# dog-qiuqiu/Yolo-FastestV2

Hardware: AMD Instinct MI355X
Metric: images/sec at 352x352 bs=256 per GPU (forward+decode+NMS) (higher is better)
Workload: dtype f32 tensors; contractions fp16x3 (two-term fp16 split operands on v_mfma_f32_16x16x32_f16, fp32 accumulate); depthwise/BN/ReLU/decode/NMS fp32 VALU; 1 GPU

## Files before the change

yolo_fastestv2_amd/csrc/yfv2_post.hip:

```cpp
#include "yfv2_internal.h"

__device__ __forceinline__ float sigmoid_f32(float x) { return __fdiv_rn(1.0f, __fadd_rn(1.0f, expf(-x))); }

template <bool SKIP = false, int MAXPER = 24>
__device__ __forceinline__ void yfv2_compact_row(const DecodeArgs& a, int b, int sc, int cc, int part, f32x4& r0, f32x4& r1,
                                                 const float (&objl)[3] = {0.f, 0.f, 0.f}, float skip_ct = 0.f) {
  const int fh = a.fh[sc], fw = a.fw[sc], hw = fh * fw;
  const int nc = a.classes;
  const int per = (nc + 3) >> 2;
  const int c_lo = part * per, c_hi = min(nc, c_lo + per);
  const float* cls = a.cls[sc] + (size_t)b * nc * hw;
  float best[3] = {0.f, 0.f, 0.f};
  int bj[3] = {0, 0, 0};
  bool need = true;
  if constexpr (SKIP) need = sigmoid_f32(objl[0]) > skip_ct || sigmoid_f32(objl[1]) > skip_ct || sigmoid_f32(objl[2]) > skip_ct;
  if (need) {
    float lv[MAXPER];
#pragma unroll
    for (int i = 0; i < MAXPER; ++i) {
      const int c = c_lo + i;
      lv[i] = cls[(unsigned)((c < c_hi ? c : (c_lo < nc ? c_lo : 0)) * hw + cc)];
    }
    float m = -INFINITY;
#pragma unroll
    for (int i = 0; i < MAXPER; ++i)
      if (c_lo + i < c_hi) m = fmaxf(m, lv[i]);
    m = fmaxf(m, __shfl_xor(m, 1));
    m = fmaxf(m, __shfl_xor(m, 2));
    float sum = 0.f;
#pragma unroll
    for (int i = 0; i < MAXPER; ++i) {
      const float e = expf(__fsub_rn(lv[i], m));
      lv[i] = e;
      if (c_lo + i < c_hi) sum = __fadd_rn(sum, e);
      if ((i & 3) == 3) __builtin_amdgcn_sched_barrier(0);
    }
    sum = __fadd_rn(sum, __shfl_xor(sum, 1));
    sum = __fadd_rn(sum, __shfl_xor(sum, 2));
    float obj3[3];
#pragma unroll
    for (int an = 0; an < 3; ++an) {
      obj3[an] = sigmoid_f32(a.obj[sc][((size_t)b * 3 + an) * hw + cc]);
      best[an] = -INFINITY;
      bj[an] = 0x7fffffff;
    }
    const float ev1 = __fdiv_rn(1.0f, sum);
    int first = 0x7fffffff, cnt = 0;
#pragma unroll
    for (int i = 0; i < MAXPER; ++i) {
      const bool near_max = c_lo + i < c_hi && lv[i] >= 0.99999904632568359375f;
      first = near_max ? min(first, c_lo + i) : first;
      cnt += near_max ? 1 : 0;
    }
    cnt += __shfl_xor(cnt, 1);
    cnt += __shfl_xor(cnt, 2);
    first = min(first, __shfl_xor(first, 1));
    first = min(first, __shfl_xor(first, 2));
    bool exact = cnt != 1;
#pragma unroll
    for (int an = 0; an < 3; ++an) {
      best[an] = __fmul_rn(ev1, obj3[an]);
      bj[an] = first;
      exact |= !(best[an] > 7.888609052210118e-31f);
    }
    if (exact) {
#pragma unroll
      for (int an = 0; an < 3; ++an) { best[an] = -INFINITY; bj[an] = 0x7fffffff; }
#pragma unroll
      for (int i = 0; i < MAXPER; ++i) {
        if (c_lo + i < c_hi) {
          const float ev = __fdiv_rn(lv[i], sum);
#pragma unroll
          for (int an = 0; an < 3; ++an) {
            const float pj = __fmul_rn(ev, obj3[an]);
            if (pj > best[an]) { best[an] = pj; bj[an] = c_lo + i; }
          }
        }
        if ((i & 3) == 3) __builtin_amdgcn_sched_barrier(0);
      }
#pragma unroll
      for (int an = 0; an < 3; ++an)
#pragma unroll
        for (int msk = 1; msk < 4; msk <<= 1) {
          const float ob_ = __shfl_xor(best[an], msk);
          const int oi = __shfl_xor(bj[an], msk);
          if (ob_ > best[an] || (ob_ == best[an] && oi < bj[an])) { best[an] = ob_; bj[an] = oi; }
        }
    }
  }
  const int an = part < 3 ? part : 0;
  const int y = cc / fw, x = cc - y * fw;
  const float* reg = a.reg[sc] + ((size_t)b * 12 + an * 4) * hw + cc;
  const float t0 = reg[0], t1 = reg[(size_t)hw], t2 = reg[(size_t)2 * hw], t3 = reg[(size_t)3 * hw];
  const float ob = a.obj[sc][((size_t)b * 3 + an) * hw + cc];
  const float st = a.stride[sc];
  const float qw = __fmul_rn(sigmoid_f32(t2), 2.0f), qh = __fmul_rn(sigmoid_f32(t3), 2.0f);
  r0 = (f32x4){__fmul_rn(__fadd_rn(__fsub_rn(__fmul_rn(sigmoid_f32(t0), 2.0f), 0.5f), (float)x), st),
               __fmul_rn(__fadd_rn(__fsub_rn(__fmul_rn(sigmoid_f32(t1), 2.0f), 0.5f), (float)y), st),
               (float)((double)__fmul_rn(qw, qw) * a.anchors[(sc * 3 + an) * 2 + 0]),
               (float)((double)__fmul_rn(qh, qh) * a.anchors[(sc * 3 + an) * 2 + 1])};
  r1 = (f32x4){sigmoid_f32(ob), part == 0 ? best[0] : (part == 1 ? best[1] : best[2]), (float)(part == 0 ? bj[0] : (part == 1 ? bj[1] : bj[2])), 0.f};
}

constexpr int DEC_CELLS = 64;
constexpr int DEC_THREADS = 256;

template <bool COMPACT, int MAXPER = 24>
__global__ __launch_bounds__(DEC_THREADS) void decode_kernel(DecodeArgs a, int blocks0, int blocks1) {
  constexpr int CELLS = MAXPER > 24 ? 32 : DEC_CELLS, THREADS = 4 * CELLS;
  extern __shared__ float stage[];
  const int per_img = blocks0 + blocks1;
  const int b = blockIdx.x / per_img;
  int blk = blockIdx.x - b * per_img;
  const int sc = blk >= blocks0 ? 1 : 0;
  if (sc) blk -= blocks0;
  const int fh = a.fh[sc], fw = a.fw[sc], hw = fh * fw;
  const int cell0 = blk * CELLS;
  const int ncell = min(CELLS, hw - cell0);
  const int nc = a.classes, rowlen = 5 + nc;
  const int tid = threadIdx.x;
  const int lc = tid >> 2, part = tid & 3;
  const int cell = cell0 + lc;
  const bool ok = lc < ncell;
  const int cc = ok ? cell : cell0;

  const int per = (nc + 3) >> 2;
  const int c_lo = part * per, c_hi = min(nc, c_lo + per);
  const float* cls = a.cls[sc] + (size_t)b * nc * hw;
  float lv[MAXPER];
#pragma unroll
  for (int i = 0; i < MAXPER; ++i) {
    const int c = c_lo + i;
    lv[i] = cls[(unsigned)((c < c_hi ? c : (c_lo < nc ? c_lo : 0)) * hw + cc)];
  }
  float m = -INFINITY;
#pragma unroll
  for (int i = 0; i < MAXPER; ++i)
    if (c_lo + i < c_hi) m = fmaxf(m, lv[i]);
  m = fmaxf(m, __shfl_xor(m, 1));
  m = fmaxf(m, __shfl_xor(m, 2));
  float sum = 0.f;
  float ev[MAXPER];
#pragma unroll
  for (int i = 0; i < MAXPER; ++i) {
    ev[i] = 0.f;
    if (c_lo + i < c_hi) {
      ev[i] = expf(__fsub_rn(lv[i], m));
      sum = __fadd_rn(sum, ev[i]);
    }
  }
  sum = __fadd_rn(sum, __shfl_xor(sum, 1));
  sum = __fadd_rn(sum, __shfl_xor(sum, 2));
#pragma unroll
  for (int i = 0; i < MAXPER; ++i) ev[i] = __fdiv_rn(ev[i], sum);

  auto box_of = [&](int an, float (&o)[5]) {
    const int y = cell / fw, x = cell - y * fw;
    const float* reg = a.reg[sc] + ((size_t)b * 12 + an * 4) * hw + cell;
    const float t0 = reg[0], t1 = reg[(size_t)hw], t2 = reg[(size_t)2 * hw], t3 = reg[(size_t)3 * hw];
    const float ob = a.obj[sc][((size_t)b * 3 + an) * hw + cell];
    const float st = a.stride[sc];
    o[0] = __fmul_rn(__fadd_rn(__fsub_rn(__fmul_rn(sigmoid_f32(t0), 2.0f), 0.5f), (float)x), st);
    o[1] = __fmul_rn(__fadd_rn(__fsub_rn(__fmul_rn(sigmoid_f32(t1), 2.0f), 0.5f), (float)y), st);
    const float qw = __fmul_rn(sigmoid_f32(t2), 2.0f), qh = __fmul_rn(sigmoid_f32(t3), 2.0f);
    o[2] = (float)((double)__fmul_rn(qw, qw) * a.anchors[(sc * 3 + an) * 2 + 0]);
    o[3] = (float)((double)__fmul_rn(qh, qh) * a.anchors[(sc * 3 + an) * 2 + 1]);
    o[4] = sigmoid_f32(ob);
  };
  const size_t row0 = (size_t)b * a.rows + (sc ? 3 * a.fh[0] * a.fw[0] : 0) + (size_t)cell0 * 3;

  if constexpr (COMPACT) {
    f32x4 r0, r1;
    yfv2_compact_row<false, MAXPER>(a, b, sc, cc, part, r0, r1);
    if (ok && part < 3) {
      float* d = a.cand + (row0 + (size_t)lc * 3 + part) * 8;
      *reinterpret_cast<f32x4*>(d) = r0;
      *reinterpret_cast<f32x4*>(d + 4) = r1;
    }
  } else {
    float* srow = stage + (size_t)lc * 3 * rowlen;
    if (ok) {
#pragma unroll
      for (int i = 0; i < MAXPER; ++i) {
        const int c = c_lo + i;
        if (c < c_hi) {
          srow[5 + c] = ev[i];
          srow[rowlen + 5 + c] = ev[i];
          srow[2 * rowlen + 5 + c] = ev[i];
        }
      }
      if (part < 3) {
        float o[5];
        box_of(part, o);
        float* d = srow + part * rowlen;
#pragma unroll
        for (int k = 0; k < 5; ++k) d[k] = o[k];
      }
    }
    __syncthreads();
    float* dst = a.boxes + row0 * rowlen;
    const int n = ncell * 3 * rowlen;
    for (int i = tid; i < n; i += THREADS) dst[i] = stage[i];
  }
}

void yfv2_launch_decode(const DecodeArgs& a, hipStream_t s) {
  const int cells = a.classes <= 96 ? DEC_CELLS : 32;
  const int b0 = (a.fh[0] * a.fw[0] + cells - 1) / cells;
  const int b1 = (a.fh[1] * a.fw[1] + cells - 1) / cells;
  const size_t lds = (size_t)cells * 3 * (5 + a.classes) * sizeof(float);
  static std::atomic<unsigned long long> lds_ok0{0}, lds_ok1{0}, lds_ok2{0}, lds_ok3{0};
  if (a.classes <= 96) {
    yfv2_allow_full_lds(reinterpret_cast<const void*>(&decode_kernel<false>), lds_ok0);
    yfv2_allow_full_lds(reinterpret_cast<const void*>(&decode_kernel<true>), lds_ok1);
    if (a.cand)
      YFV2_LAUNCH(decode_kernel<true>, dim3(a.B * (b0 + b1)), dim3(DEC_THREADS), 0, s, a, b0, b1);
    else
      YFV2_LAUNCH(decode_kernel<false>, dim3(a.B * (b0 + b1)), dim3(DEC_THREADS), lds, s, a, b0, b1);
  } else {
    yfv2_allow_full_lds(reinterpret_cast<const void*>(&decode_kernel<false, 64>), lds_ok2);
    yfv2_allow_full_lds(reinterpret_cast<const void*>(&decode_kernel<true, 64>), lds_ok3);
    if (a.cand)
      YFV2_LAUNCH((decode_kernel<true, 64>), dim3(a.B * (b0 + b1)), dim3(4 * cells), 0, s, a, b0, b1);
    else
      YFV2_LAUNCH((decode_kernel<false, 64>), dim3(a.B * (b0 + b1)), dim3(4 * cells), lds, s, a, b0, b1);
  }
}
bool yfv2_post_fusable(int classes, int rows) { return classes <= 96 && rows <= 2048; }
int yfv2_nms_max_rows() { return 4096; }

constexpr int NMS_THREADS = 1024;
constexpr int NMS_NQ = NMS_THREADS / 64;
constexpr int NMS_CAP = 2048;
constexpr int NMS_MAX_DET = 300;

#define NMS_STAMP(i) do { if (a.trace && blockIdx.x == 0 && threadIdx.x == 0) a.trace[i] = (long long)__builtin_readcyclecounter(); } while (0)
template <int SRC, int KPT = 2>
__global__ __launch_bounds__(NMS_THREADS) void nms_kernel(NmsArgs a, DecodeArgs dec) {
  constexpr bool COMPACT = SRC >= 1;
  constexpr int CAP = KPT * NMS_THREADS;
  static_assert(KPT == 2 || (KPT == 4 && SRC != 2), "two keys per thread, or four without the in-LDS decode");
  extern __shared__ __attribute__((aligned(16))) float crow[];
  __shared__ unsigned long long key[CAP];
  __shared__ __attribute__((aligned(16))) float geo[(KPT == 2 ? 7 : 5) * CAP];
  unsigned long long* const key2 = reinterpret_cast<unsigned long long*>(geo);
  float* const bx1 = geo + (KPT == 2 ? 2 * CAP : 0);
  float* const by1 = bx1 + CAP; float* const bx2 = by1 + CAP; float* const by2 = bx2 + CAP; float* const area = by2 + CAP;
  __shared__ unsigned char supp[CAP];
  __shared__ unsigned char cls_of_row[CAP];
  __shared__ int keep[NMS_MAX_DET];
  __shared__ float kx1[NMS_MAX_DET], kx2[NMS_MAX_DET];
  __shared__ unsigned long long pmask[NMS_NQ][64];
  __shared__ int n_cand, n_keep, n_obj;

  const int tid = threadIdx.x, b = blockIdx.x;
  const int rowlen = COMPACT ? 8 : 5 + a.nc;
  const float* img = SRC == 2 ? crow : a.boxes + (size_t)b * a.rows * rowlen;
  const float ct = a.conf_thres;
  NMS_STAMP(0);
  if constexpr (SRC == 2) {
    constexpr int CPP = NMS_THREADS / 4;
    const int hw0 = dec.fh[0] * dec.fw[0], hw1 = dec.fh[1] * dec.fw[1];
    const int np0 = (hw0 + CPP - 1) / CPP, np = np0 + (hw1 + CPP - 1) / CPP;
    const int part = tid & 3;
    auto obj_of = [&](int ps, float (&o)[3]) {
      const int sc = ps < np0 ? 0 : 1, hw = sc ? hw1 : hw0;
      const int cell = (ps - (sc ? np0 : 0)) * CPP + (tid >> 2);
      const int cc = cell < hw ? cell : hw - 1;
#pragma unroll
      for (int an = 0; an < 3; ++an) o[an] = ps < np ? dec.obj[sc][((size_t)b * 3 + an) * hw + cc] : 0.f;
    };
    float ocur[3], onxt[3];
    obj_of(0, ocur);
    for (int ps = 0; ps < np; ++ps) {
      obj_of(ps + 1, onxt);
      const int sc = ps < np0 ? 0 : 1, hw = sc ? hw1 : hw0;
      const int row_base = sc ? 3 * hw0 : 0;
      const int cell = (ps - (sc ? np0 : 0)) * CPP + (tid >> 2);
      const bool ok = cell < hw;
      f32x4 r0, r1;
      yfv2_compact_row<true>(dec, b, sc, ok ? cell : hw - 1, part, r0, r1, ocur, ct);
      if (ok && part < 3) {
        float* d = crow + (size_t)(row_base + cell * 3 + part) * 8;
        *reinterpret_cast<f32x4*>(d) = r0;
        *reinterpret_cast<f32x4*>(d + 4) = r1;
      }
#pragma unroll
      for (int an = 0; an < 3; ++an) ocur[an] = onxt[an];
    }
    __syncthreads();
  }
  NMS_STAMP(1);
  unsigned short* cand_row = reinterpret_cast<unsigned short*>(bx1);
  if (tid == 0) { n_cand = 0; n_keep = 0; n_obj = 0; }
  __syncthreads();

  if constexpr (COMPACT) {
    for (int n0 = 0; n0 < a.rows; n0 += NMS_THREADS) {
      const int n = n0 + tid;
      f32x4 t = {0.f, 0.f, 0.f, 0.f};
      if (n < a.rows) t = *reinterpret_cast<const f32x4*>(img + (size_t)n * 8 + 4);
      const bool pass = n < a.rows && t[0] > ct && t[1] > ct;
      const unsigned long long m = __ballot(pass);
      int base = 0;
      if ((tid & 63) == 0 && m) base = atomicAdd(&n_cand, (int)__popcll(m));
      base = __shfl(base, 0);
      if (pass) {
        const int slot = base + (int)__popcll(m & ((1ull << (tid & 63)) - 1ull));
        key[slot] = ((unsigned long long)__float_as_uint(t[1]) << 32) | (unsigned long long)(0xFFFFFFFFu - (unsigned)n);
        cls_of_row[n] = (unsigned char)(int)t[2];
      }
    }
  } else {
    for (int n0 = 0; n0 < a.rows; n0 += NMS_THREADS) {
      const int n = n0 + tid;
      const bool pass = n < a.rows && img[(size_t)n * rowlen + 4] > ct;
      const unsigned long long m = __ballot(pass);
      int base = 0;
      if ((tid & 63) == 0 && m) base = atomicAdd(&n_obj, (int)__popcll(m));
      base = __shfl(base, 0);
      if (pass) cand_row[base + (int)__popcll(m & ((1ull << (tid & 63)) - 1ull))] = (unsigned short)n;
    }
    __syncthreads();
    {
      const int l16 = tid & 15, grp = tid >> 4, ngrp = NMS_THREADS >> 4;
      const int nobj = n_obj;
      for (int q = grp; q < nobj; q += ngrp) {
        const int n = cand_row[q];
        const float* r = img + (size_t)n * rowlen;
        const float obj = r[4];
        float best = -INFINITY;
        int bj = 0x7fffffff;
        for (int j = l16; j < a.nc; j += 16) {
          const float pj = __fmul_rn(r[5 + j], obj);
          if (pj > best) { best = pj; bj = j; }
        }
#pragma unroll
        for (int m = 1; m < 16; m <<= 1) {
          const float ob = __shfl_xor(best, m, 16);
          const int oj = __shfl_xor(bj, m, 16);
          if (ob > best || (ob == best && oj < bj)) { best = ob; bj = oj; }
        }
        if (l16 == 0 && best > ct) {
          bool hit = true;
          if (a.classes) {
            hit = false;
            for (int k = 0; k < a.n_classes; ++k) hit |= (a.classes[k] == bj);
          }
          if (hit) {
            const int slot = atomicAdd(&n_cand, 1);
            key[slot] = ((unsigned long long)__float_as_uint(best) << 32) | (unsigned long long)(0xFFFFFFFFu - (unsigned)n);
            cls_of_row[n] = (unsigned char)bj;
          }
        }
      }
    }
  }
  __syncthreads();
  NMS_STAMP(2);
  const int n = n_cand;
  if (n == 0) {
    if (tid == 0) a.count[b] = 0;
    return;
  }

  int np2 = 1;
  while (np2 < n) np2 <<= 1;
  for (int i = n + tid; i < np2; i += NMS_THREADS) key[i] = 0ull;
  __syncthreads();
  if constexpr (KPT == 2) {
    static_assert(NMS_CAP == 2 * NMS_THREADS, "two keys per thread");
    const int i0 = tid, i1 = tid + NMS_THREADS;
    unsigned long long k0 = i0 < np2 ? key[i0] : 0ull, k1 = i1 < np2 ? key[i1] : 0ull;
    auto cx = [](unsigned long long x, unsigned long long y, bool take_max) { return take_max == (x > y) ? x : y; };
    int pb = 0;
    for (int k = 2; k <= np2; k <<= 1) {
      for (int j = k >> 1; j > 0; j >>= 1) {
        const bool d0 = (i0 & k) == 0, d1 = (i1 & k) == 0;
        if (j >= NMS_THREADS) {
          const unsigned long long hi = k0 > k1 ? k0 : k1, lo = k0 > k1 ? k1 : k0;
          k0 = d0 ? hi : lo; k1 = d0 ? lo : hi;
        } else if (j >= 64) {
          unsigned long long* buf = pb ? key2 : key;
          buf[i0] = k0; buf[i1] = k1;
          __syncthreads();
          const unsigned long long y0 = buf[i0 ^ j], y1 = buf[i1 ^ j];
          const bool low = (i0 & j) == 0;
          k0 = cx(k0, y0, low == d0); k1 = cx(k1, y1, low == d1);
          pb ^= 1;
        } else {
          const unsigned long long y0 = __shfl_xor(k0, j), y1 = __shfl_xor(k1, j);
          const bool low = (i0 & j) == 0;
          k0 = cx(k0, y0, low == d0); k1 = cx(k1, y1, low == d1);
        }
      }
    }
    __syncthreads();
    if (i0 < np2) key[i0] = k0;
    if (i1 < np2) key[i1] = k1;
    __syncthreads();
  } else {
    unsigned long long k[KPT];
#pragma unroll
    for (int r = 0; r < KPT; ++r) { const int i = tid + r * NMS_THREADS; k[r] = i < np2 ? key[i] : 0ull; }
    auto cx = [](unsigned long long x, unsigned long long y, bool take_max) { return take_max == (x > y) ? x : y; };
    int pb = 0;
    for (int kk = 2; kk <= np2; kk <<= 1) {
      for (int j = kk >> 1; j > 0; j >>= 1) {
        if (j >= NMS_THREADS) {
          const int jr = j / NMS_THREADS;
#pragma unroll
          for (int r = 0; r < KPT; ++r) {
            if ((r & jr) == 0) {
              const int r2 = r | jr;
              const bool desc = ((tid + r * NMS_THREADS) & kk) == 0;
              const unsigned long long hi = k[r] > k[r2] ? k[r] : k[r2], lo = k[r] > k[r2] ? k[r2] : k[r];
              k[r] = desc ? hi : lo; k[r2] = desc ? lo : hi;
            }
          }
        } else if (j >= 64) {
          unsigned long long* buf = pb ? key2 : key;
#pragma unroll
          for (int r = 0; r < KPT; ++r) buf[tid + r * NMS_THREADS] = k[r];
          __syncthreads();
          const bool low = (tid & j) == 0;
#pragma unroll
          for (int r = 0; r < KPT; ++r) {
            const int i = tid + r * NMS_THREADS;
            k[r] = cx(k[r], buf[i ^ j], low == ((i & kk) == 0));
          }
          pb ^= 1;
        } else {
          const bool low = (tid & j) == 0;
#pragma unroll
          for (int r = 0; r < KPT; ++r) {
            const int i = tid + r * NMS_THREADS;
            k[r] = cx(k[r], __shfl_xor(k[r], j), low == ((i & kk) == 0));
          }
        }
      }
    }
    __syncthreads();
#pragma unroll
    for (int r = 0; r < KPT; ++r) { const int i = tid + r * NMS_THREADS; if (i < np2) key[i] = k[r]; }
    __syncthreads();
  }

  NMS_STAMP(3);
  for (int i = tid; i < n; i += NMS_THREADS) {
    const unsigned row = 0xFFFFFFFFu - (unsigned)(key[i] & 0xFFFFFFFFull);
    const float* r = img + (size_t)row * rowlen;
    const float cx = r[0], cy = r[1], hw_ = __fdiv_rn(r[2], 2.0f), hh = __fdiv_rn(r[3], 2.0f);
    const float c = __fmul_rn((float)cls_of_row[row], 4096.0f);
    const float x1 = __fadd_rn(__fsub_rn(cx, hw_), c), y1 = __fadd_rn(__fsub_rn(cy, hh), c);
    const float x2 = __fadd_rn(__fadd_rn(cx, hw_), c), y2 = __fadd_rn(__fadd_rn(cy, hh), c);
    bx1[i] = x1; by1[i] = y1; bx2[i] = x2; by2[i] = y2;
    area[i] = __fmul_rn(__fsub_rn(x2, x1), __fsub_rn(y2, y1));
    supp[i] = 0;
  }
  __syncthreads();

  NMS_STAMP(4);
  const bool thr_nonneg = a.iou_thres >= 0.0;
  auto overlaps = [&](int i, int j) -> bool {
    const float xx1 = fmaxf(bx1[i], bx1[j]), xx2 = fminf(bx2[i], bx2[j]);
    if (thr_nonneg && !(xx2 > xx1)) return false;
    const float yy1 = fmaxf(by1[i], by1[j]), yy2 = fminf(by2[i], by2[j]);
    const float w = fmaxf(0.0f, __fsub_rn(xx2, xx1)), h = fmaxf(0.0f, __fsub_rn(yy2, yy1));
    const float inter = __fmul_rn(w, h);
    const float ovr = __fdiv_rn(inter, __fsub_rn(__fadd_rn(area[i], area[j]), inter));
    return (double)ovr > a.iou_thres;
  };
  const int j = tid & 63, q = tid >> 6;
  long long t_tests = 0, t_walk = 0, t_bar = 0; int n_chunks = 0;
  const bool tr = a.trace && blockIdx.x == 0 && tid == 0;
  for (int c0 = 0; c0 < n; c0 += 64) {
    const int nk = n_keep;
    if (nk >= NMS_MAX_DET) break;
    const long long ts0 = tr ? (long long)__builtin_readcyclecounter() : 0;
    const int m = min(64, n - c0);
    unsigned long long bits = 0ull;
    {
      constexpr int KMAX = (NMS_MAX_DET + NMS_NQ - 1) / NMS_NQ;
      constexpr int PER = 64 / NMS_NQ;
      auto lane_f = [](float v, int l) { return __builtin_bit_cast(float, __builtin_amdgcn_readlane(__builtin_bit_cast(int, v), l)); };
      const int cj = c0 + j;
      const bool live = j < m;
      const float jx1 = live ? bx1[cj] : INFINITY, jx2 = live ? bx2[cj] : -INFINITY;
      const int kl = q + NMS_NQ * j;
      const bool kv = j < KMAX && kl < nk;
      const float rk1 = kv ? kx1[kl] : INFINITY, rk2 = kv ? kx2[kl] : -INFINITY;
      unsigned cand = 0u;
#pragma unroll
      for (int t = 0; t < KMAX; ++t) {
        const float a1 = lane_f(rk1, t), a2 = lane_f(rk2, t);
        if (q + NMS_NQ * t < nk && (!thr_nonneg || fminf(a2, jx2) > fmaxf(a1, jx1))) cand |= 1u << t;
      }
      unsigned icand = 0u;
#pragma unroll
      for (int c = 0; c < PER; ++c) {
        const int i = PER * q + c;
        const float a1 = lane_f(jx1, i), a2 = lane_f(jx2, i);
        if (i < j && (!thr_nonneg || fminf(a2, jx2) > fmaxf(a1, jx1))) icand |= 1u << c;
      }
      if (live) {
        while (cand) {
          const int t = __builtin_ctz(cand);
          cand &= cand - 1u;
          if (overlaps(keep[q + NMS_NQ * t], cj)) { supp[cj] = 1; break; }
        }
        while (icand) {
          const int c = __builtin_ctz(icand);
          icand &= icand - 1u;
          if (overlaps(c0 + PER * q + c, cj)) bits |= 1ull << (PER * q + c);
        }
      }
    }
    pmask[q][j] = bits;
    const long long ts1 = tr ? (long long)__builtin_readcyclecounter() : 0;
    __syncthreads();
    const long long ts2 = tr ? (long long)__builtin_readcyclecounter() : 0;
    if (tid < 64) {
      unsigned long long S = 0ull;
#pragma unroll
      for (int qq = 0; qq < NMS_NQ; ++qq) S |= pmask[qq][tid];
      const bool alive = tid < m && !supp[c0 + tid];
      const unsigned long long alive_mask = __ballot(alive);
      unsigned long long kmask = alive_mask;
      for (int it = 0; it < 64; ++it) {
        const unsigned long long k2 = __ballot(alive && !(S & kmask));
        if (k2 == kmask) break;
        kmask = k2;
      }
      if ((kmask >> tid) & 1ull) {
        const int pos = nk + __popcll(kmask & ((1ull << tid) - 1ull));
        if (pos < NMS_MAX_DET) { keep[pos] = c0 + tid; kx1[pos] = bx1[c0 + tid]; kx2[pos] = bx2[c0 + tid]; }
      }
      if (tid == 0) n_keep = min(NMS_MAX_DET, nk + __popcll(kmask));
    }
    const long long ts3 = tr ? (long long)__builtin_readcyclecounter() : 0;
    __syncthreads();
    if (tr) { const long long ts4 = (long long)__builtin_readcyclecounter(); t_tests += ts1 - ts0; t_walk += ts3 - ts2; t_bar += (ts2 - ts1) + (ts4 - ts3); ++n_chunks; }
  }
  if (tr) { a.trace[9] = n_chunks; a.trace[10] = t_tests; a.trace[11] = t_walk; a.trace[12] = t_bar; }
  __syncthreads();
  NMS_STAMP(5);
  const int kept = n_keep;

  for (int k = tid; k < kept; k += NMS_THREADS) {
    const int i = keep[k];
    const unsigned long long kk = key[i];
    const unsigned row = 0xFFFFFFFFu - (unsigned)(kk & 0xFFFFFFFFull);
    const float* r = img + (size_t)row * rowlen;
    const float cx = r[0], cy = r[1], hw_ = __fdiv_rn(r[2], 2.0f), hh = __fdiv_rn(r[3], 2.0f);
    float* d = a.dets + ((size_t)b * NMS_MAX_DET + k) * 6;
    d[0] = __fsub_rn(cx, hw_); d[1] = __fsub_rn(cy, hh);
    d[2] = __fadd_rn(cx, hw_); d[3] = __fadd_rn(cy, hh);
    d[4] = __uint_as_float((unsigned)(kk >> 32));
    d[5] = (float)cls_of_row[row];
    a.idx[(size_t)b * NMS_MAX_DET + k] = (int)row;
  }
  if (tid == 0) a.count[b] = kept;
  NMS_STAMP(6);
  if (a.trace && blockIdx.x == 0 && tid == 0) { a.trace[7] = n; a.trace[8] = kept; }
}

void yfv2_launch_nms(const NmsArgs& a, hipStream_t s) {
  const DecodeArgs none{};
  if (a.rows <= NMS_CAP) {
    if (a.compact)
      YFV2_LAUNCH(nms_kernel<1>, dim3(a.B), dim3(NMS_THREADS), 0, s, a, none);
    else
      YFV2_LAUNCH(nms_kernel<0>, dim3(a.B), dim3(NMS_THREADS), 0, s, a, none);
  } else {
    if (a.compact)
      YFV2_LAUNCH((nms_kernel<1, 4>), dim3(a.B), dim3(NMS_THREADS), 0, s, a, none);
    else
      YFV2_LAUNCH((nms_kernel<0, 4>), dim3(a.B), dim3(NMS_THREADS), 0, s, a, none);
  }
}

void yfv2_launch_decode_nms(const DecodeArgs& d, const NmsArgs& a, hipStream_t s) {
  static std::atomic<unsigned long long> done{0};
  int dev = 0;
  if (hipGetDevice(&dev) != hipSuccess || dev < 0 || dev > 63) dev = 0;
  if (!(done.load() & (1ull << dev))) {
    (void)hipFuncSetAttribute(reinterpret_cast<const void*>(&nms_kernel<2>), hipFuncAttributeMaxDynamicSharedMemorySize, NMS_CAP * 8 * (int)sizeof(float));
    done.fetch_or(1ull << dev);
  }
  YFV2_LAUNCH(nms_kernel<2>, dim3(a.B), dim3(NMS_THREADS), (size_t)a.rows * 8 * sizeof(float), s, a, d);
}

__global__ __launch_bounds__(64) void stats_kernel(StatsArgs a) {
  __shared__ float tx1[STATS_MAX_TARGETS], ty1[STATS_MAX_TARGETS], tx2[STATS_MAX_TARGETS], ty2[STATS_MAX_TARGETS], tlab[STATS_MAX_TARGETS];
  __shared__ int tdone[STATS_MAX_TARGETS];
  const int b = blockIdx.x, lane = threadIdx.x;
  int nt = 0;
  for (int t0 = 0; t0 < a.T; t0 += 64) {
    const int t = t0 + lane;
    const bool mine = t < a.T && a.targets[(size_t)t * 6] == (float)b;
    const unsigned long long m = __ballot(mine);
    if (mine) {
      const int pos = nt + __popcll(m & ((1ull << lane) - 1ull));
      if (pos < STATS_MAX_TARGETS) {
        tlab[pos] = a.targets[(size_t)t * 6 + 1];
        tx1[pos] = a.targets[(size_t)t * 6 + 2]; ty1[pos] = a.targets[(size_t)t * 6 + 3];
        tx2[pos] = a.targets[(size_t)t * 6 + 4]; ty2[pos] = a.targets[(size_t)t * 6 + 5];
        tdone[pos] = 0;
      }
    }
    nt += __popcll(m);
  }
  if (nt > STATS_MAX_TARGETS) { if (lane == 0) *a.overflow = 1; nt = STATS_MAX_TARGETS; }
  __syncthreads();
  const int n = a.count[b];
  int* tp = a.tp + (size_t)b * NMS_MAX_DET;
  for (int i = lane; i < NMS_MAX_DET; i += 64) tp[i] = 0;
  if (nt == 0) return;
  const float thr = a.iou_thres;
  int matched = 0;
  for (int i = 0; i < n && matched < nt; ++i) {
    const float* d = a.dets + ((size_t)b * NMS_MAX_DET + i) * 6;
    const float bx1 = d[0], by1 = d[1], bx2 = d[2], by2 = d[3], lab = d[5];
    const float barea = __fmul_rn(__fadd_rn(__fsub_rn(bx2, bx1), 1.f), __fadd_rn(__fsub_rn(by2, by1), 1.f));
    bool has = false;
    float best = -1.f;
    int bidx = 0x7fffffff;
    for (int t = lane; t < nt; t += 64) {
      has |= tlab[t] == lab;
      const float ix1 = fmaxf(bx1, tx1[t]), iy1 = fmaxf(by1, ty1[t]), ix2 = fminf(bx2, tx2[t]), iy2 = fminf(by2, ty2[t]);
      const float iw = fmaxf(__fadd_rn(__fsub_rn(ix2, ix1), 1.f), 0.f), ih = fmaxf(__fadd_rn(__fsub_rn(iy2, iy1), 1.f), 0.f);
      const float inter = __fmul_rn(iw, ih);
      const float tarea = __fmul_rn(__fadd_rn(__fsub_rn(tx2[t], tx1[t]), 1.f), __fadd_rn(__fsub_rn(ty2[t], ty1[t]), 1.f));
      const float iou = __fdiv_rn(inter, __fadd_rn(__fsub_rn(__fadd_rn(barea, tarea), inter), 1e-16f));
      if (iou > best) { best = iou; bidx = t; }
    }
    if (__ballot(has) == 0ull) continue;
#pragma unroll
    for (int off = 32; off > 0; off >>= 1) {
      const float ob = __shfl_xor(best, off);
      const int oi = __shfl_xor(bidx, off);
      if (ob > best || (ob == best && oi < bidx)) { best = ob; bidx = oi; }
    }
    if (best >= thr && tdone[bidx] == 0) {
      if (lane == 0) { tp[i] = 1; tdone[bidx] = 1; }
      ++matched;
    }
    __syncthreads();
  }
}

void yfv2_launch_stats(const StatsArgs& a, hipStream_t s) { YFV2_LAUNCH(stats_kernel, dim3(a.B), dim3(64), 0, s, a); }
```

Before: 458,200 images/s.

## Use DPP/permlane lane exchanges in decode and NMS sort, restructure in-NMS decode per wave

```diff
diff --git a/yolo_fastestv2_amd/csrc/yfv2_post.hip b/yolo_fastestv2_amd/csrc/yfv2_post.hip
--- a/yolo_fastestv2_amd/csrc/yfv2_post.hip
+++ b/yolo_fastestv2_amd/csrc/yfv2_post.hip
@@ -1,19 +1,32 @@
 #include "yfv2_internal.h"
 
 __device__ __forceinline__ float sigmoid_f32(float x) { return __fdiv_rn(1.0f, __fadd_rn(1.0f, expf(-x))); }
+
+template <int J>
+__device__ __forceinline__ int quad_xor(int v) {
+  static_assert(J == 1 || J == 2, "quad_perm exchange inside four lanes");
+  return __builtin_amdgcn_update_dpp(0, v, J == 1 ? 0xB1 : 0x4E, 0xF, 0xF, false);
+}
+template <int J> __device__ __forceinline__ float quad_xor(float v) { return __int_as_float(quad_xor<J>(__float_as_int(v))); }
 
 template <bool SKIP = false, int MAXPER = 24>
 __device__ __forceinline__ void yfv2_compact_row(const DecodeArgs& a, int b, int sc, int cc, int part, f32x4& r0, f32x4& r1,
-                                                 const float (&objl)[3] = {0.f, 0.f, 0.f}, float skip_ct = 0.f) {
+                                                 float objl = 0.f, float skip_ct = 0.f) {
   const int fh = a.fh[sc], fw = a.fw[sc], hw = fh * fw;
   const int nc = a.classes;
   const int per = (nc + 3) >> 2;
   const int c_lo = part * per, c_hi = min(nc, c_lo + per);
+  const int an = part < 3 ? part : 0;
   const float* cls = a.cls[sc] + (size_t)b * nc * hw;
-  float best[3] = {0.f, 0.f, 0.f};
-  int bj[3] = {0, 0, 0};
-  bool need = true;
-  if constexpr (SKIP) need = sigmoid_f32(objl[0]) > skip_ct || sigmoid_f32(objl[1]) > skip_ct || sigmoid_f32(objl[2]) > skip_ct;
+  const float so = sigmoid_f32(SKIP ? objl : a.obj[sc][((size_t)b * 3 + an) * hw + cc]);
+  float conf = 0.f;
+  int cj = 0;
+  int need = 1;
+  if constexpr (SKIP) {
+    need = so > skip_ct ? 1 : 0;
+    need |= quad_xor<1>(need);
+    need |= quad_xor<2>(need);
+  }
   if (need) {
     float lv[MAXPER];
 #pragma unroll
@@ -25,8 +38,8 @@
 #pragma unroll
     for (int i = 0; i < MAXPER; ++i)
       if (c_lo + i < c_hi) m = fmaxf(m, lv[i]);
-    m = fmaxf(m, __shfl_xor(m, 1));
-    m = fmaxf(m, __shfl_xor(m, 2));
+    m = fmaxf(m, quad_xor<1>(m));
+    m = fmaxf(m, quad_xor<2>(m));
     float sum = 0.f;
 #pragma unroll
     for (int i = 0; i < MAXPER; ++i) {
@@ -35,15 +48,8 @@
       if (c_lo + i < c_hi) sum = __fadd_rn(sum, e);
       if ((i & 3) == 3) __builtin_amdgcn_sched_barrier(0);
     }
-    sum = __fadd_rn(sum, __shfl_xor(sum, 1));
-    sum = __fadd_rn(sum, __shfl_xor(sum, 2));
-    float obj3[3];
-#pragma unroll
-    for (int an = 0; an < 3; ++an) {
-      obj3[an] = sigmoid_f32(a.obj[sc][((size_t)b * 3 + an) * hw + cc]);
-      best[an] = -INFINITY;
-      bj[an] = 0x7fffffff;
-    }
+    sum = __fadd_rn(sum, quad_xor<1>(sum));
+    sum = __fadd_rn(sum, quad_xor<2>(sum));
     const float ev1 = __fdiv_rn(1.0f, sum);
     int first = 0x7fffffff, cnt = 0;
 #pragma unroll
@@ -52,54 +58,64 @@
       first = near_max ? min(first, c_lo + i) : first;
       cnt += near_max ? 1 : 0;
     }
-    cnt += __shfl_xor(cnt, 1);
-    cnt += __shfl_xor(cnt, 2);
-    first = min(first, __shfl_xor(first, 1));
-    first = min(first, __shfl_xor(first, 2));
-    bool exact = cnt != 1;
-#pragma unroll
-    for (int an = 0; an < 3; ++an) {
-      best[an] = __fmul_rn(ev1, obj3[an]);
-      bj[an] = first;
-      exact |= !(best[an] > 7.888609052210118e-31f);
-    }
+    cnt += quad_xor<1>(cnt);
+    cnt += quad_xor<2>(cnt);
+    first = min(first, quad_xor<1>(first));
+    first = min(first, quad_xor<2>(first));
+    conf = __fmul_rn(ev1, so);
+    cj = first;
+    int exact = cnt != 1 || !(conf > 7.888609052210118e-31f) ? 1 : 0;
+    exact |= quad_xor<1>(exact);
+    exact |= quad_xor<2>(exact);
     if (exact) {
-#pragma unroll
-      for (int an = 0; an < 3; ++an) { best[an] = -INFINITY; bj[an] = 0x7fffffff; }
+      const float o1 = quad_xor<1>(so), o2 = quad_xor<2>(so), o3 = quad_xor<1>(o2);
+      float obj3[3], best[3];
+      int bj[3];
+#pragma unroll
+      for (int k = 0; k < 3; ++k) {
+        const int d = k ^ part;
+        obj3[k] = d == 0 ? so : (d == 1 ? o1 : (d == 2 ? o2 : o3));
+        best[k] = -INFINITY;
+        bj[k] = 0x7fffffff;
+      }
 #pragma unroll
       for (int i = 0; i < MAXPER; ++i) {
         if (c_lo + i < c_hi) {
           const float ev = __fdiv_rn(lv[i], sum);
 #pragma unroll
-          for (int an = 0; an < 3; ++an) {
-            const float pj = __fmul_rn(ev, obj3[an]);
-            if (pj > best[an]) { best[an] = pj; bj[an] = c_lo + i; }
+          for (int k = 0; k < 3; ++k) {
+            const float pj = __fmul_rn(ev, obj3[k]);
+            if (pj > best[k]) { best[k] = pj; bj[k] = c_lo + i; }
           }
         }
         if ((i & 3) == 3) __builtin_amdgcn_sched_barrier(0);
       }
 #pragma unroll
-      for (int an = 0; an < 3; ++an)
-#pragma unroll
-        for (int msk = 1; msk < 4; msk <<= 1) {
-          const float ob_ = __shfl_xor(best[an], msk);
-          const int oi = __shfl_xor(bj[an], msk);
-          if (ob_ > best[an] || (ob_ == best[an] && oi < bj[an])) { best[an] = ob_; bj[an] = oi; }
-        }
-    }
-  }
-  const int an = part < 3 ? part : 0;
-  const int y = cc / fw, x = cc - y * fw;
-  const float* reg = a.reg[sc] + ((size_t)b * 12 + an * 4) * hw + cc;
-  const float t0 = reg[0], t1 = reg[(size_t)hw], t2 = reg[(size_t)2 * hw], t3 = reg[(size_t)3 * hw];
-  const float ob = a.obj[sc][((size_t)b * 3 + an) * hw + cc];
-  const float st = a.stride[sc];
-  const float qw = __fmul_rn(sigmoid_f32(t2), 2.0f), qh = __fmul_rn(sigmoid_f32(t3), 2.0f);
-  r0 = (f32x4){__fmul_rn(__fadd_rn(__fsub_rn(__fmul_rn(sigmoid_f32(t0), 2.0f), 0.5f), (float)x), st),
-               __fmul_rn(__fadd_rn(__fsub_rn(__fmul_rn(sigmoid_f32(t1), 2.0f), 0.5f), (float)y), st),
-               (float)((double)__fmul_rn(qw, qw) * a.anchors[(sc * 3 + an) * 2 + 0]),
-               (float)((double)__fmul_rn(qh, qh) * a.anchors[(sc * 3 + an) * 2 + 1])};
-  r1 = (f32x4){sigmoid_f32(ob), part == 0 ? best[0] : (part == 1 ? best[1] : best[2]), (float)(part == 0 ? bj[0] : (part == 1 ? bj[1] : bj[2])), 0.f};
+      for (int k = 0; k < 3; ++k) {
+        float ob_ = quad_xor<1>(best[k]);
+        int oi = quad_xor<1>(bj[k]);
+        if (ob_ > best[k] || (ob_ == best[k] && oi < bj[k])) { best[k] = ob_; bj[k] = oi; }
+        ob_ = quad_xor<2>(best[k]);
+        oi = quad_xor<2>(bj[k]);
+        if (ob_ > best[k] || (ob_ == best[k] && oi < bj[k])) { best[k] = ob_; bj[k] = oi; }
+      }
+      conf = part == 0 ? best[0] : (part == 1 ? best[1] : best[2]);
+      cj = part == 0 ? bj[0] : (part == 1 ? bj[1] : bj[2]);
+    }
+  }
+  r0 = (f32x4){0.f, 0.f, 0.f, 0.f};
+  if (part < 3) {
+    const int y = cc / fw, x = cc - y * fw;
+    const float* reg = a.reg[sc] + ((size_t)b * 12 + an * 4) * hw + cc;
+    const float t0 = reg[0], t1 = reg[(size_t)hw], t2 = reg[(size_t)2 * hw], t3 = reg[(size_t)3 * hw];
+    const float st = a.stride[sc];
+    const float qw = __fmul_rn(sigmoid_f32(t2), 2.0f), qh = __fmul_rn(sigmoid_f32(t3), 2.0f);
+    r0 = (f32x4){__fmul_rn(__fadd_rn(__fsub_rn(__fmul_rn(sigmoid_f32(t0), 2.0f), 0.5f), (float)x), st),
+                 __fmul_rn(__fadd_rn(__fsub_rn(__fmul_rn(sigmoid_f32(t1), 2.0f), 0.5f), (float)y), st),
+                 (float)((double)__fmul_rn(qw, qw) * a.anchors[(sc * 3 + an) * 2 + 0]),
+                 (float)((double)__fmul_rn(qh, qh) * a.anchors[(sc * 3 + an) * 2 + 1])};
+  }
+  r1 = (f32x4){so, conf, (float)cj, 0.f};
 }
 
 constexpr int DEC_CELLS = 64;
@@ -234,6 +250,88 @@
 constexpr int NMS_CAP = 2048;
 constexpr int NMS_MAX_DET = 300;
 
+__device__ __forceinline__ unsigned xor_sel_mask() {
+  const int l = (int)(threadIdx.x & 63);
+  const bool s4 = __builtin_amdgcn_update_dpp(0, l, 0x124, 0xF, 0xF, false) == (l ^ 4);
+  const auto p16 = __builtin_amdgcn_permlane16_swap(l, l, false, false);
+  const auto p32 = __builtin_amdgcn_permlane32_swap(l, l, false, false);
+  return (s4 ? 4u : 0u) | ((int)p16[0] == (l ^ 16) ? 16u : 0u) | ((int)p32[0] == (l ^ 32) ? 32u : 0u);
+}
+template <int J>
+__device__ __forceinline__ unsigned xor_lane32(unsigned v, unsigned sel) {
+  const int x = (int)v;
+  if constexpr (J == 1 || J == 2) return (unsigned)quad_xor<J>(x);
+  else if constexpr (J == 8) return (unsigned)__builtin_amdgcn_update_dpp(0, x, 0x128, 0xF, 0xF, false);
+  else if constexpr (J == 4) {
+    const int r4 = __builtin_amdgcn_update_dpp(0, x, 0x124, 0xF, 0xF, false), r12 = __builtin_amdgcn_update_dpp(0, x, 0x12C, 0xF, 0xF, false);
+    return (unsigned)((sel & 4u) ? r4 : r12);
+  } else if constexpr (J == 16) {
+    const auto p = __builtin_amdgcn_permlane16_swap(x, x, false, false);
+    return (unsigned)((sel & 16u) ? (int)p[0] : (int)p[1]);
+  } else {
+    static_assert(J == 32, "lane distance");
+    const auto p = __builtin_amdgcn_permlane32_swap(x, x, false, false);
+    return (unsigned)((sel & 32u) ? (int)p[0] : (int)p[1]);
+  }
+}
+template <int J>
+__device__ __forceinline__ unsigned long long xor_lane64(unsigned long long v, unsigned sel) {
+  return ((unsigned long long)xor_lane32<J>((unsigned)(v >> 32), sel) << 32) | xor_lane32<J>((unsigned)v, sel);
+}
+
+template <int KPT>
+__device__ __forceinline__ void bitonic_sort(unsigned long long* key, unsigned long long* key2, int np2, int tid) {
+  const unsigned sel = xor_sel_mask();
+  unsigned long long k[KPT];
+#pragma unroll
+  for (int r = 0; r < KPT; ++r) { const int i = tid + r * NMS_THREADS; k[r] = i < np2 ? key[i] : 0ull; }
+  auto cx = [](unsigned long long x, unsigned long long y, bool take_max) { return take_max == (x > y) ? x : y; };
+  int pb = 0;
+  for (int kk = 2; kk <= np2; kk <<= 1) {
+    int j = kk >> 1;
+    for (; j >= 64; j >>= 1) {
+      if (j >= NMS_THREADS) {
+        const int jr = j / NMS_THREADS;
+#pragma unroll
+        for (int r = 0; r < KPT; ++r) {
+          if ((r & jr) == 0 && (r | jr) < KPT) {
+            const int r2 = r | jr;
+            const bool desc = ((tid + r * NMS_THREADS) & kk) == 0;
+            const unsigned long long hi = k[r] > k[r2] ? k[r] : k[r2], lo = k[r] > k[r2] ? k[r2] : k[r];
+            k[r] = desc ? hi : lo; k[r2] = desc ? lo : hi;
+          }
+        }
+      } else {
+        unsigned long long* buf = pb ? key2 : key;
+#pragma unroll
+        for (int r = 0; r < KPT; ++r) buf[tid + r * NMS_THREADS] = k[r];
+        __syncthreads();
+        const bool low = (tid & j) == 0;
+#pragma unroll
+        for (int r = 0; r < KPT; ++r) {
+          const int i = tid + r * NMS_THREADS;
+          k[r] = cx(k[r], buf[i ^ j], low == ((i & kk) == 0));
+        }
+        pb ^= 1;
+      }
+    }
+#define YFV2_SORT_STEP(J)                                                                   \
+    if (J < kk) {                                                                           \
+      const bool low = (tid & J) == 0;                                                      \
+      _Pragma("unroll") for (int r = 0; r < KPT; ++r) {                                     \
+        const int i = tid + r * NMS_THREADS;                                                \
+        k[r] = cx(k[r], xor_lane64<J>(k[r], sel), low == ((i & kk) == 0));                 \
+      }                                                                                     \
+    }
+    YFV2_SORT_STEP(32) YFV2_SORT_STEP(16) YFV2_SORT_STEP(8) YFV2_SORT_STEP(4) YFV2_SORT_STEP(2) YFV2_SORT_STEP(1)
+#undef YFV2_SORT_STEP
+  }
+  __syncthreads();
+#pragma unroll
+  for (int r = 0; r < KPT; ++r) { const int i = tid + r * NMS_THREADS; if (i < np2) key[i] = k[r]; }
+  __syncthreads();
+}
+
 #define NMS_STAMP(i) do { if (a.trace && blockIdx.x == 0 && threadIdx.x == 0) a.trace[i] = (long long)__builtin_readcyclecounter(); } while (0)
 template <int SRC, int KPT = 2>
 __global__ __launch_bounds__(NMS_THREADS) void nms_kernel(NmsArgs a, DecodeArgs dec) {
@@ -259,24 +357,23 @@
   const float ct = a.conf_thres;
   NMS_STAMP(0);
   if constexpr (SRC == 2) {
-    constexpr int CPP = NMS_THREADS / 4;
+    constexpr int WC = 16;
     const int hw0 = dec.fh[0] * dec.fw[0], hw1 = dec.fh[1] * dec.fw[1];
-    const int np0 = (hw0 + CPP - 1) / CPP, np = np0 + (hw1 + CPP - 1) / CPP;
-    const int part = tid & 3;
-    auto obj_of = [&](int ps, float (&o)[3]) {
-      const int sc = ps < np0 ? 0 : 1, hw = sc ? hw1 : hw0;
-      const int cell = (ps - (sc ? np0 : 0)) * CPP + (tid >> 2);
-      const int cc = cell < hw ? cell : hw - 1;
-#pragma unroll
-      for (int an = 0; an < 3; ++an) o[an] = ps < np ? dec.obj[sc][((size_t)b * 3 + an) * hw + cc] : 0.f;
+    const int nw0 = (hw0 + WC - 1) / WC, nw = nw0 + (hw1 + WC - 1) / WC;
+    const int wv = __builtin_amdgcn_readfirstlane(tid >> 6);
+    const int part = tid & 3, an = part < 3 ? part : 0;
+    auto obj_of = [&](int w) -> float {
+      if (w >= nw) return 0.f;
+      const int sc = w >= nw0 ? 1 : 0, hw = sc ? hw1 : hw0;
+      const int cell = (w - (sc ? nw0 : 0)) * WC + ((tid & 63) >> 2);
+      return dec.obj[sc][((size_t)b * 3 + an) * hw + (cell < hw ? cell : hw - 1)];
     };
-    float ocur[3], onxt[3];
-    obj_of(0, ocur);
-    for (int ps = 0; ps < np; ++ps) {
-      obj_of(ps + 1, onxt);
-      const int sc = ps < np0 ? 0 : 1, hw = sc ? hw1 : hw0;
+    float ocur = obj_of(wv);
+    for (int w = wv; w < nw; w += NMS_NQ) {
+      const float onxt = obj_of(w + NMS_NQ);
+      const int sc = w >= nw0 ? 1 : 0, hw = sc ? hw1 : hw0;
       const int row_base = sc ? 3 * hw0 : 0;
-      const int cell = (ps - (sc ? np0 : 0)) * CPP + (tid >> 2);
+      const int cell = (w - (sc ? nw0 : 0)) * WC + ((tid & 63) >> 2);
       const bool ok = cell < hw;
       f32x4 r0, r1;
       yfv2_compact_row<true>(dec, b, sc, ok ? cell : hw - 1, part, r0, r1, ocur, ct);
@@ -285,8 +382,7 @@
         *reinterpret_cast<f32x4*>(d) = r0;
         *reinterpret_cast<f32x4*>(d + 4) = r1;
       }
-#pragma unroll
-      for (int an = 0; an < 3; ++an) ocur[an] = onxt[an];
+      ocur = onxt;
     }
     __syncthreads();
   }
@@ -368,83 +464,8 @@
   while (np2 < n) np2 <<= 1;
   for (int i = n + tid; i < np2; i += NMS_THREADS) key[i] = 0ull;
   __syncthreads();
-  if constexpr (KPT == 2) {
-    static_assert(NMS_CAP == 2 * NMS_THREADS, "two keys per thread");
-    const int i0 = tid, i1 = tid + NMS_THREADS;
-    unsigned long long k0 = i0 < np2 ? key[i0] : 0ull, k1 = i1 < np2 ? key[i1] : 0ull;
-    auto cx = [](unsigned long long x, unsigned long long y, bool take_max) { return take_max == (x > y) ? x : y; };
-    int pb = 0;
-    for (int k = 2; k <= np2; k <<= 1) {
-      for (int j = k >> 1; j > 0; j >>= 1) {
-        const bool d0 = (i0 & k) == 0, d1 = (i1 & k) == 0;
-        if (j >= NMS_THREADS) {
-          const unsigned long long hi = k0 > k1 ? k0 : k1, lo = k0 > k1 ? k1 : k0;
-          k0 = d0 ? hi : lo; k1 = d0 ? lo : hi;
-        } else if (j >= 64) {
-          unsigned long long* buf = pb ? key2 : key;
-          buf[i0] = k0; buf[i1] = k1;
-          __syncthreads();
-          const unsigned long long y0 = buf[i0 ^ j], y1 = buf[i1 ^ j];
-          const bool low = (i0 & j) == 0;
-          k0 = cx(k0, y0, low == d0); k1 = cx(k1, y1, low == d1);
-          pb ^= 1;
-        } else {
-          const unsigned long long y0 = __shfl_xor(k0, j), y1 = __shfl_xor(k1, j);
-          const bool low = (i0 & j) == 0;
-          k0 = cx(k0, y0, low == d0); k1 = cx(k1, y1, low == d1);
-        }
-      }
-    }
-    __syncthreads();
-    if (i0 < np2) key[i0] = k0;
-    if (i1 < np2) key[i1] = k1;
-    __syncthreads();
-  } else {
-    unsigned long long k[KPT];
-#pragma unroll
-    for (int r = 0; r < KPT; ++r) { const int i = tid + r * NMS_THREADS; k[r] = i < np2 ? key[i] : 0ull; }
-    auto cx = [](unsigned long long x, unsigned long long y, bool take_max) { return take_max == (x > y) ? x : y; };
-    int pb = 0;
-    for (int kk = 2; kk <= np2; kk <<= 1) {
-      for (int j = kk >> 1; j > 0; j >>= 1) {
-        if (j >= NMS_THREADS) {
-          const int jr = j / NMS_THREADS;
-#pragma unroll
-          for (int r = 0; r < KPT; ++r) {
-            if ((r & jr) == 0) {
-              const int r2 = r | jr;
-              const bool desc = ((tid + r * NMS_THREADS) & kk) == 0;
-              const unsigned long long hi = k[r] > k[r2] ? k[r] : k[r2], lo = k[r] > k[r2] ? k[r2] : k[r];
-              k[r] = desc ? hi : lo; k[r2] = desc ? lo : hi;
-            }
-          }
-        } else if (j >= 64) {
-          unsigned long long* buf = pb ? key2 : key;
-#pragma unroll
-          for (int r = 0; r < KPT; ++r) buf[tid + r * NMS_THREADS] = k[r];
-          __syncthreads();
-          const bool low = (tid & j) == 0;
-#pragma unroll
-          for (int r = 0; r < KPT; ++r) {
-            const int i = tid + r * NMS_THREADS;
-            k[r] = cx(k[r], buf[i ^ j], low == ((i & kk) == 0));
-          }
-          pb ^= 1;
-        } else {
-          const bool low = (tid & j) == 0;
-#pragma unroll
-          for (int r = 0; r < KPT; ++r) {
-            const int i = tid + r * NMS_THREADS;
-            k[r] = cx(k[r], __shfl_xor(k[r], j), low == ((i & kk) == 0));
-          }
-        }
-      }
-    }
-    __syncthreads();
-#pragma unroll
-    for (int r = 0; r < KPT; ++r) { const int i = tid + r * NMS_THREADS; if (i < np2) key[i] = k[r]; }
-    __syncthreads();
-  }
+  if (np2 <= NMS_THREADS) bitonic_sort<1>(key, key2, np2, tid);
+  else bitonic_sort<KPT>(key, key2, np2, tid);
 
   NMS_STAMP(3);
   for (int i = tid; i < n; i += NMS_THREADS) {
```

Result: faster. 468,800 images/s, median of 6 (+2.3%).
